# EPFL-VILAB/MultiMAE

Measured on NVIDIA H100. Metric: MultiMAE-B pretrain samples/sec @ bs=128/GPU, higher is better.
Workload: dtype bf16

## Files before the change

include/multimae_b200.h:

```cpp
#ifndef MULTIMAE_B200_H_
#define MULTIMAE_B200_H_

#include <stdint.h>

#ifdef __cplusplus
extern "C" {
#endif

#define MMAE_ABI_VERSION 11

int mmae_abi_version(void);
const char* mmae_last_error(void);
int64_t mmae_launch_count(void);

int mmae_profile_gemm(int enable);
int mmae_profile_gemm_read(double* flops, double* ms, int64_t* launches);
int64_t mmae_profile_gemm_dump(char* buf_host, int64_t capacity);

typedef struct mmae_gemm_epilogue {
  float alpha;
  int act;
  int accumulate;
  int reserved;
  const float* bias;
  const float* residual;
  const void* dgelu_z;
  void* preact_bf16;
  float* out_f32;
  void* out_bf16;
  int64_t ld_residual, ld_dgelu_z, ld_preact, ld_out_f32, ld_out_bf16;
} mmae_gemm_epilogue;

int mmae_gemm_set_variant(int variant);
int mmae_gemm_set_tma_store(int enable);
int mmae_set_pdl(int enable);
int mmae_set_sm_budget(int sms);
int mmae_set_wgrad_stream(int enable);

int mmae_gemm_bf16(const void* A, int64_t lda, int a_mn_major, const void* B, int64_t ldb, int b_mn_major,
                   int M, int N, int K, int split_k, const mmae_gemm_epilogue* ep, void* stream);

int mmae_cast_f32_to_bf16(const float* src, void* dst_bf16, int64_t n, void* stream);
int mmae_cast_colsum_f32(const float* src, int64_t ld_src, void* dst_bf16, int64_t ld_dst, float* colsum,
                         int M, int N, void* stream);
int mmae_colsum_bf16(const void* src_bf16, int64_t ld_src, float* colsum, int M, int N, void* stream);
int mmae_gelu_bf16(const void* z, void* io, int64_t n, int backward, void* stream);
int mmae_dgelu_colsum_bf16(const void* z, void* dz, int64_t ld, float* colsum, int M, int N, void* stream);
int mmae_set_fuse_gelu(int enable);
int mmae_add_bf16_f32(const float* x, const void* y_bf16, float* out, int64_t n, void* stream);
int mmae_transpose_bf16(const void* src, int64_t ld_src, void* dst, int64_t ld_dst, int M, int N, void* stream);

int mmae_layernorm_forward(const float* x, int64_t ldx, const float* gamma, const float* beta, void* y_bf16,
                           int64_t ldy, float* y_f32, int64_t ldyf, float* mean, float* rstd, int M, int D,
                           float eps, void* stream);
int mmae_add_layernorm_forward(const float* x, int64_t ldx, const void* addend_bf16, int64_t ldadd, float* x_sum,
                               int64_t ldsum, const float* gamma, const float* beta, void* y_bf16, int64_t ldy,
                               float* mean, float* rstd, int M, int D, float eps, void* stream);
int mmae_layernorm_backward(const void* dy, int dy_is_bf16, int64_t lddy, const float* x, int64_t ldx,
                            const float* mean, const float* rstd, const float* gamma, const float* dx_resid,
                            int64_t ldr, float* dx, int64_t lddx, float* dgamma, float* dbeta, int M, int D,
                            void* stream);

int mmae_layernorm_backward_ex(const void* dy, int dy_is_bf16, int64_t lddy, const float* x, int64_t ldx,
// ... 263 lines not shown
```

multimae_b200/_lib.py:

```python
import ctypes
import os

_HERE = os.path.dirname(os.path.abspath(__file__))
LIB_PATH = os.path.join(_HERE, "libmultimae_b200.so")

c_void_p = ctypes.c_void_p
c_int = ctypes.c_int
c_i64 = ctypes.c_int64
c_float = ctypes.c_float


class GemmEpilogue(ctypes.Structure):
    _fields_ = [
        ("alpha", c_float),
        ("act", c_int),
        ("accumulate", c_int),
        ("reserved", c_int),
        ("bias", c_void_p),
        ("residual", c_void_p),
        ("dgelu_z", c_void_p),
        ("preact_bf16", c_void_p),
        ("out_f32", c_void_p),
        ("out_bf16", c_void_p),
        ("ld_residual", c_i64),
        ("ld_dgelu_z", c_i64),
        ("ld_preact", c_i64),
        ("ld_out_f32", c_i64),
        ("ld_out_bf16", c_i64),
    ]


MAX_TASKS = 8
c_float_p = c_void_p
POS_MODES = {"bicubic": 0, "bilinear": 1}


class EmbedLayout(ctypes.Structure):
    _fields_ = [
        ("num_tasks", c_int),
        ("grid_h", c_int * MAX_TASKS), ("grid_w", c_int * MAX_TASKS),
        ("tok_offset", c_int * (MAX_TASKS + 1)),
        ("k_offset", c_int * (MAX_TASKS + 1)),
        ("patch", c_int * MAX_TASKS), ("channels", c_int * MAX_TASKS),
        ("is_semseg", c_int * MAX_TASKS), ("num_classes", c_int * MAX_TASKS),
    ]


class EmbedInputs(ctypes.Structure):
    _fields_ = [("data", c_void_p * MAX_TASKS), ("class_emb", c_void_p * MAX_TASKS)]


class EmbedParams(ctypes.Structure):
    _fields_ = [("weight", c_void_p * MAX_TASKS), ("bias", c_void_p * MAX_TASKS), ("pos", c_void_p * MAX_TASKS),
                ("global_tokens", c_void_p)]


class EmbedGrads(ctypes.Structure):
    _fields_ = [("weight", c_void_p * MAX_TASKS), ("bias", c_void_p * MAX_TASKS), ("class_emb", c_void_p * MAX_TASKS),
                ("global_tokens", c_void_p)]


# ... 253 lines not shown
```

multimae_b200/csrc/gemm_wgmma.cu:

```cuda
#include <algorithm>
#include <cstdlib>

#include "common.cuh"
#include "../../include/multimae_b200.h"

namespace mmae {

void count_launch();
bool gemm_profile_begin(cudaStream_t st, double flops, int M, int N, int K, int flags);
void gemm_profile_end(cudaStream_t st);

namespace {

constexpr int BM = 128;
constexpr int BK = 64;
constexpr int WG_K = 16;
constexpr int GEMM_THREADS = 384;

struct GemmParams {
  int M, N, K;
  int num_kb;
  int kb_per_split;
  int tiles_n;
  int tiles_m;
  int splits;
  int tma_store;
  mmae_gemm_epilogue ep;
};

template <int BN>
struct GemmCfg {
  static constexpr int STAGES = BN == 256 ? 4 : (BN == 192 ? 4 : (BN == 128 ? 6 : 8));
  static constexpr int A_BYTES = BM * BK * 2;
  static constexpr int B_BYTES = BN * BK * 2;
  static constexpr int STAGE_BYTES = A_BYTES + B_BYTES;
  static constexpr int EPI_BOX_BYTES = 64 * 32 * 4;
  static constexpr int EPI_OFFSET = STAGES * STAGE_BYTES;
  static constexpr int BAR_OFFSET = EPI_OFFSET + 2 * 2 * EPI_BOX_BYTES;
  static constexpr int TOTAL = BAR_OFFSET + 256 + 1024;
  static_assert(TOTAL <= 232448, "GEMM exceeds the 227 KB shared-memory limit");
};

struct WorkItem {
  int m0, n0, split, kb_begin, nkb;
};

template <int BN, int CL>
__device__ __forceinline__ WorkItem decode_item(int item, const GemmParams& p, int rank) {
  WorkItem w;
  const int rest = item / p.tiles_n;
  w.n0 = (item - rest * p.tiles_n) * BN;
  w.split = rest / p.tiles_m;
  w.m0 = ((rest - w.split * p.tiles_m) * CL + rank) * BM;
  w.kb_begin = w.split * p.kb_per_split;
  w.nkb = min(p.kb_per_split, p.num_kb - w.kb_begin);
  return w;
}

__device__ __forceinline__ void red_add_v2(float* addr, float a, float b) {
  asm volatile("red.global.add.v2.f32 [%0], {%1, %2};" ::"l"(addr), "f"(a), "f"(b) : "memory");
}

__device__ __forceinline__ void epilogue_pair(float v0, float v1, int row, int n, const GemmParams& p, bool first_split,
                                              bool atomic_out) {
  const mmae_gemm_epilogue& ep = p.ep;
  v0 *= ep.alpha;
  v1 *= ep.alpha;
  if (ep.bias && first_split) {
    const float2 b = __ldg(reinterpret_cast<const float2*>(ep.bias + n));
    v0 += b.x;
    v1 += b.y;
  }
  if (ep.preact_bf16)
    *reinterpret_cast<uint32_t*>(reinterpret_cast<bf16*>(ep.preact_bf16) + int64_t(row) * ep.ld_preact + n) = pack_bf16x2(v0, v1);
  if (ep.act == 1) {
    v0 = gelu_erf(v0);
    v1 = gelu_erf(v1);
  }
  if (ep.dgelu_z) {
    const uint32_t z = __ldg(reinterpret_cast<const unsigned int*>(reinterpret_cast<const bf16*>(ep.dgelu_z) +
                                                                   int64_t(row) * ep.ld_dgelu_z + n));
    const float2 zf = unpack_bf16x2(z);
    v0 *= dgelu_erf(zf.x);
    v1 *= dgelu_erf(zf.y);
  }
  if (ep.residual && first_split) {
    const float2 r = __ldg(reinterpret_cast<const float2*>(ep.residual + int64_t(row) * ep.ld_residual + n));
    v0 += r.x;
    v1 += r.y;
  }
  if (ep.out_f32) {
    float* dst = ep.out_f32 + int64_t(row) * ep.ld_out_f32 + n;
    if (atomic_out) red_add_v2(dst, v0, v1);
    else *reinterpret_cast<float2*>(dst) = make_float2(v0, v1);
  }
  if (ep.out_bf16)
    *reinterpret_cast<uint32_t*>(reinterpret_cast<bf16*>(ep.out_bf16) + int64_t(row) * ep.ld_out_bf16 + n) = pack_bf16x2(v0, v1);
}

template <typename T>
__device__ __forceinline__ void stage_pair(uint8_t* box, int r, int c, float v0, float v1) {
  T* b = reinterpret_cast<T*>(box);
  if constexpr (sizeof(T) == 4) *reinterpret_cast<float2*>(b + r * 32 + c) = make_float2(v0, v1);
  else *reinterpret_cast<uint32_t*>(b + r * 32 + c) = pack_bf16x2(v0, v1);
}

template <int BN, int CL, bool A_MN, bool B_MN>
__global__ void __launch_bounds__(GEMM_THREADS, 1)
    gemm_bf16_kernel(const __grid_constant__ CUtensorMap tmA, const __grid_constant__ CUtensorMap tmB,
                     const __grid_constant__ CUtensorMap tmC, const GemmParams p) {
  pdl_launch_dependents();
  using C = GemmCfg<BN>;
  constexpr int STAGES = C::STAGES;
  constexpr int BH = BN / CL;
  static_assert(!B_MN || BH % 64 == 0, "MN-major B is loaded in 64-column chunks");

  extern __shared__ uint8_t smem_raw[];
  const uint32_t raw_addr = smem_u32(smem_raw);
  uint8_t* smem = smem_raw + ((1024u - (raw_addr & 1023u)) & 1023u);
  uint64_t* full_bar = reinterpret_cast<uint64_t*>(smem + C::BAR_OFFSET);
  uint64_t* empty_bar = full_bar + STAGES;

  const int wg = threadIdx.x >> 7;
  const int rank = CL > 1 ? int(cluster_ctarank()) : 0;
  const int num_items = p.tiles_n * p.tiles_m * p.splits;
  const int first_item = blockIdx.x / CL;
  const int item_stride = gridDim.x / CL;

  if (threadIdx.x == 0) {
    tma_prefetch_desc(&tmA);
    tma_prefetch_desc(&tmB);
    if (p.tma_store) tma_prefetch_desc(&tmC);
#pragma unroll
    for (int s = 0; s < STAGES; ++s) {
      mbar_init(&full_bar[s], 1);
      mbar_init(&empty_bar[s], 2 * CL);
    }
    fence_barrier_init();
  }
  __syncthreads();
  if constexpr (CL > 1) cluster_sync_all();
  pdl_wait();

  if (wg == 0) {
    setmaxnreg_dec<40>();
    if (threadIdx.x == 0) {
      uint32_t it = 0;
      for (int item = first_item; item < num_items; item += item_stride) {
        const WorkItem w = decode_item<BN, CL>(item, p, rank);
        for (int kb = 0; kb < w.nkb; ++kb, ++it) {
          const int s = it % STAGES;
          const uint32_t ph = (it / STAGES) & 1;
          mbar_wait(&empty_bar[s], ph ^ 1u);
          mbar_expect_tx(&full_bar[s], C::STAGE_BYTES);
          uint8_t* sA = smem + s * C::STAGE_BYTES;
          uint8_t* sB = sA + C::A_BYTES;
          const int k0 = (w.kb_begin + kb) * BK;
          if constexpr (!A_MN) {
            tma_load_2d(sA, &tmA, &full_bar[s], k0, w.m0);
          } else {
#pragma unroll
            for (int c = 0; c < BM / 64; ++c) tma_load_2d(sA + c * (64 * BK * 2), &tmA, &full_bar[s], w.m0 + c * 64, k0);
          }
          if constexpr (CL == 1) {
            if constexpr (!B_MN) {
              tma_load_2d(sB, &tmB, &full_bar[s], k0, w.n0);
            } else {
#pragma unroll
              for (int c = 0; c < BN / 64; ++c) tma_load_2d(sB + c * (64 * BK * 2), &tmB, &full_bar[s], w.n0 + c * 64, k0);
            }
          } else {
            if constexpr (!B_MN) {
              tma_load_2d_multicast(sB + rank * BH * 128, &tmB, &full_bar[s], k0, w.n0 + rank * BH, 0x3);
            } else {
#pragma unroll
              for (int c = 0; c < BH / 64; ++c)
                tma_load_2d_multicast(sB + (rank * (BH / 64) + c) * (64 * BK * 2), &tmB, &full_bar[s],
                                      w.n0 + rank * BH + c * 64, k0, 0x3);
            }
          }
        }
      }
    }
  } else {
    setmaxnreg_inc<232>();
    const int cw = wg - 1;
    const int t = threadIdx.x & 127;
    const int rl = (t >> 5) * 16 + ((t & 31) >> 2);
    uint8_t* epi = smem + C::EPI_OFFSET + cw * (2 * C::EPI_BOX_BYTES);
    const bool atomic_out = p.ep.accumulate != 0 || p.splits > 1;
    uint32_t it = 0;
    uint32_t boxes = 0;
    auto release = [&](int s) {
      if (t == 0) {
        if constexpr (CL == 1) mbar_arrive(&empty_bar[s]);
        else
          for (int r = 0; r < CL; ++r) mbar_arrive_cluster(mapa_u32(smem_u32(&empty_bar[s]), uint32_t(r)));
      }
    };
    float acc[BN / 2];

    for (int item = first_item; item < num_items; item += item_stride) {
      const WorkItem w = decode_item<BN, CL>(item, p, rank);
      for (int kb = 0; kb < w.nkb; ++kb, ++it) {
        const int s = it % STAGES;
        const uint32_t ph = (it / STAGES) & 1;
        mbar_wait(&full_bar[s], ph);
        const uint32_t a_addr = smem_u32(smem + s * C::STAGE_BYTES) + cw * (64 * BK * 2);
        const uint32_t b_addr = smem_u32(smem + s * C::STAGE_BYTES) + C::A_BYTES;
#pragma unroll
        for (int i = 0; i < BN / 2; ++i) reg_fence(acc[i]);
        wgmma_fence();
#pragma unroll
        for (int j = 0; j < BK / WG_K; ++j) {
          const uint32_t sd = (kb | j) != 0 ? 1u : 0u;
          const uint64_t da = A_MN ? gmma_desc_sw128(a_addr + j * (WG_K * 128), 64 * BK * 2, 1024)
                                   : gmma_desc_sw128(a_addr + j * (WG_K * 2), 16, 1024);
          const uint64_t db = B_MN ? gmma_desc_sw128(b_addr + j * (WG_K * 128), 64 * BK * 2, 1024)
                                   : gmma_desc_sw128(b_addr + j * (WG_K * 2), 16, 1024);
          if constexpr (BN == 256) wgmma_m64n256k16<A_MN ? 1 : 0, B_MN ? 1 : 0>(acc, da, db, sd);
          else if constexpr (BN == 192) wgmma_m64n192k16<A_MN ? 1 : 0, B_MN ? 1 : 0>(acc, da, db, sd);
          else if constexpr (BN == 128) wgmma_m64n128k16<A_MN ? 1 : 0, B_MN ? 1 : 0>(acc, da, db, sd);
          else wgmma_m64n64k16<A_MN ? 1 : 0, B_MN ? 1 : 0>(acc, da, db, sd);
        }
        wgmma_commit();
#pragma unroll
        for (int i = 0; i < BN / 2; ++i) reg_fence(acc[i]);
        wgmma_wait<1>();
        if (kb > 0) release((it - 1) % STAGES);
      }
      wgmma_wait<0>();
#pragma unroll
      for (int i = 0; i < BN / 2; ++i) reg_fence(acc[i]);
      release((it - 1) % STAGES);

      const int row_a = w.m0 + cw * 64 + rl;
      const int row_b = row_a + 8;
      const bool first_split = w.split == 0;
      if (p.tma_store) {
        const float* bias = first_split ? p.ep.bias : nullptr;
        const bool bf16_out = p.tma_store == 1;
#pragma unroll
        for (int b = 0; b < BN / 32; ++b) {
          if (w.n0 + b * 32 >= p.N) break;
          uint8_t* box = bf16_out ? epi + (boxes & 3) * (C::EPI_BOX_BYTES / 2) : epi + (boxes & 1) * C::EPI_BOX_BYTES;
          if (t == 0) {
            if (bf16_out) bulk_wait_read<3>();
            else bulk_wait_read<1>();
          }
          asm volatile("bar.sync %0, 128;" ::"r"(2 + cw) : "memory");
#pragma unroll
          for (int jj = 0; jj < 4; ++jj) {
            const int j = 4 * b + jj;
            const int c = jj * 8 + 2 * (t & 3);
            float v[4] = {acc[4 * j] * p.ep.alpha, acc[4 * j + 1] * p.ep.alpha, acc[4 * j + 2] * p.ep.alpha,
                          acc[4 * j + 3] * p.ep.alpha};
            if (bias && w.n0 + b * 32 + c < p.N) {
              const float2 bb = __ldg(reinterpret_cast<const float2*>(bias + w.n0 + b * 32 + c));
              v[0] += bb.x; v[1] += bb.y; v[2] += bb.x; v[3] += bb.y;
            }
            if (p.ep.act == 1) {
#pragma unroll
              for (int i = 0; i < 4; ++i) v[i] = gelu_erf(v[i]);
            }
            if (bf16_out) {
              stage_pair<bf16>(box, rl, c, v[0], v[1]);
              stage_pair<bf16>(box, rl + 8, c, v[2], v[3]);
            } else {
              stage_pair<float>(box, rl, c, v[0], v[1]);
              stage_pair<float>(box, rl + 8, c, v[2], v[3]);
            }
          }
          fence_proxy_async_smem();
          asm volatile("bar.sync %0, 128;" ::"r"(2 + cw) : "memory");
          if (t == 0) {
            if (p.tma_store == 3) tma_reduce_add_2d(&tmC, box, w.n0 + b * 32, w.m0 + cw * 64);
            else tma_store_2d(&tmC, box, w.n0 + b * 32, w.m0 + cw * 64);
            bulk_commit_group();
          }
          ++boxes;
        }
      } else {
#pragma unroll
        for (int j = 0; j < BN / 8; ++j) {
          if (w.n0 + j * 8 >= p.N) break;
          const int n = w.n0 + j * 8 + 2 * (t & 3);
          if (row_a < p.M) epilogue_pair(acc[4 * j], acc[4 * j + 1], row_a, n, p, first_split, atomic_out);
          if (row_b < p.M) epilogue_pair(acc[4 * j + 2], acc[4 * j + 3], row_b, n, p, first_split, atomic_out);
        }
      }
    }
    if (t == 0 && p.tma_store) bulk_wait_all();
  }
  if constexpr (CL > 1) cluster_sync_all();
}

template <int BN, int CL, bool A_MN, bool B_MN>
int launch_gemm(const CUtensorMap& tmA, const CUtensorMap& tmB, const CUtensorMap& tmC, const GemmParams& p,
                cudaStream_t stream) {
  using C = GemmCfg<BN>;
  auto kern = gemm_bf16_kernel<BN, CL, A_MN, B_MN>;
  cudaLaunchConfig_t cfg;
  memset(&cfg, 0, sizeof(cfg));
  cfg.blockDim = dim3(GEMM_THREADS);
  cfg.dynamicSmemBytes = C::TOTAL;
  cfg.stream = stream;
  cudaLaunchAttribute attr[2];
  attr[0].id = cudaLaunchAttributeClusterDimension;
  attr[0].val.clusterDim.x = CL;
  attr[0].val.clusterDim.y = 1;
  attr[0].val.clusterDim.z = 1;
  attr[1].id = cudaLaunchAttributeProgrammaticStreamSerialization;
  attr[1].val.programmaticStreamSerializationAllowed = 1;
  cfg.attrs = attr;
  cfg.numAttrs = 1;
  static int resident = 0;
  if (resident == 0) {
    MMAE_CUDA_OK(cudaFuncSetAttribute(kern, cudaFuncAttributeMaxDynamicSharedMemorySize, C::TOTAL));
    if constexpr (CL > 1) {
      cfg.gridDim = dim3(CL);
      MMAE_CUDA_OK(cudaOccupancyMaxActiveClusters(&resident, kern, &cfg));
    } else {
      int dev = 0, sms = 0;
      MMAE_CUDA_OK(cudaGetDevice(&dev));
      MMAE_CUDA_OK(cudaDeviceGetAttribute(&sms, cudaDevAttrMultiProcessorCount, dev));
      resident = sms;
    }
    MMAE_CHECK(resident > 0, MMAE_ERR_CUDA, "mmae_gemm_bf16: the GEMM kernel does not fit on an SM");
  }
  const int items = p.tiles_n * p.tiles_m * p.splits;
  const int slots = std::min(resident, std::max(1, sm_count() / CL));
  cfg.gridDim = dim3(std::min(items, slots) * CL);
  const bool prof = gemm_profile_begin(stream, 2.0 * p.M * p.N * p.K, p.M, p.N, p.K,
                                       (A_MN ? 1 : 0) | (B_MN ? 2 : 0) | (p.splits << 8));
  if constexpr (CL == 1) {
    cfg.attrs = attr + 1;
    cfg.numAttrs = pdl_enabled() ? 1 : 0;
  } else {
    cfg.numAttrs = pdl_enabled() ? 2 : 1;
  }
  MMAE_CUDA_OK(cudaLaunchKernelEx(&cfg, kern, tmA, tmB, tmC, p));
  if (prof) gemm_profile_end(stream);
  count_launch();
  MMAE_LAUNCH_OK();
  return MMAE_OK;
}

}
}

using namespace mmae;

static int g_gemm_variant = []() {
  const char* e = getenv("MMAE_GEMM_VARIANT");
  const int v = e ? atoi(e) : -1;
  return v >= -1 && v <= 6 ? v : -1;
}();
static int g_gemm_tma_store = []() {
  const char* e = getenv("MMAE_GEMM_TMA_STORE");
  return e ? (atoi(e) != 0) : 1;
}();

extern "C" int mmae_gemm_set_variant(int variant) {
  MMAE_CHECK(variant >= -1 && variant <= 6, MMAE_ERR_ARG, "mmae_gemm_set_variant: %d (-1 .. 6)", variant);
  g_gemm_variant = variant;
  return MMAE_OK;
}

extern "C" int mmae_gemm_set_tma_store(int enable) {
  g_gemm_tma_store = enable != 0;
  return MMAE_OK;
}

static int variant_bn(int v) { return v == 0 ? 64 : (v == 1 || v == 6) ? 128 : (v == 3 || v == 5) ? 192 : 256; }
// ... 25 lines not shown
    for (int i = 0; i < nvar; ++i) {
      const int v = variant >= 0 ? variant : cand_var[i];
      const int bn = variant_bn(v), cl = v >= 4 ? 2 : 1;
      if (variant < 0 && bn > 128 && N < bn) continue;
      const long tiles = long(ceil_div(tm, cl)) * ceil_div(N, bn);
      const int slots = std::max(1, sms / cl);
      const int s_lo = split_k > 0 ? split_k : 1;
      const int s_hi = split_k > 0 ? split_k : std::max(1, num_kb / MIN_KB_PER_SPLIT);
      for (int s = s_lo; s <= s_hi; ++s) {
        const int kbps = ceil_div(num_kb, std::min(s, num_kb));
        const long rounds = (tiles * ceil_div(num_kb, kbps) + slots - 1) / slots;
        const long cost = rounds * (bn + 40) * cl * (kbps + KB_PER_ITEM_FIXED);
        if (best_cost < 0 || cost < best_cost) {
          best_cost = cost;
          best_split = s;
          best_var = v;
        }
      }
    }
    split_k = best_split;
    variant = best_var;
  }
  if (split_k > num_kb) split_k = num_kb;
  const int kb_per_split = ceil_div(num_kb, split_k);
  split_k = ceil_div(num_kb, kb_per_split);
  if (split_k > 1 || ep->accumulate) {
    MMAE_CHECK(ep->out_f32 && !ep->out_bf16 && !ep->preact_bf16 && !ep->dgelu_z && ep->act == 0, MMAE_ERR_ARG,
               "mmae_gemm_bf16: split-K / accumulate supports only a linear fp32 epilogue");
  }
#define MMAE_LD_OK(ptr, ld) (!(ptr) || ((ld) % 8 == 0 && (reinterpret_cast<uintptr_t>(ptr) & 15) == 0))
  MMAE_CHECK(MMAE_LD_OK(ep->residual, ep->ld_residual) && MMAE_LD_OK(ep->dgelu_z, ep->ld_dgelu_z) &&
                 MMAE_LD_OK(ep->preact_bf16, ep->ld_preact) && MMAE_LD_OK(ep->out_f32, ep->ld_out_f32) &&
                 MMAE_LD_OK(ep->out_bf16, ep->ld_out_bf16) &&
                 (!ep->bias || (reinterpret_cast<uintptr_t>(ep->bias) & 15) == 0),
             MMAE_ERR_ARG, "mmae_gemm_bf16: epilogue tensors need 16-byte alignment and ld %% 8 == 0");
#undef MMAE_LD_OK

  if (variant == 5 && b_mn_major) variant = 4;
  const int BNsel = variant_bn(variant);
  const int CLsel = variant >= 4 ? 2 : 1;

  CUtensorMap tmA, tmB;
  int rc;
  if (!a_mn_major) {
    rc = make_tmap_2d_bf16(&tmA, A, (uint64_t)M, (uint64_t)K, (uint64_t)lda, BK, BM);
  } else {
    MMAE_CHECK(M % 8 == 0, MMAE_ERR_ARG, "mmae_gemm_bf16: MN-major A needs M %% 8 == 0");
    rc = make_tmap_2d_bf16(&tmA, A, (uint64_t)K, (uint64_t)M, (uint64_t)lda, 64, BK);
  }
  if (rc) return rc;
  if (!b_mn_major) {
    rc = make_tmap_2d_bf16(&tmB, B, (uint64_t)N, (uint64_t)K, (uint64_t)ldb, BK, BNsel / CLsel);
  } else {
    rc = make_tmap_2d_bf16(&tmB, B, (uint64_t)K, (uint64_t)N, (uint64_t)ldb, 64, BK);
  }
  if (rc) return rc;

  GemmParams p;
  p.M = M; p.N = N; p.K = K;
  p.num_kb = num_kb;
  p.kb_per_split = kb_per_split;
  p.tiles_n = ceil_div(N, BNsel);
  p.tiles_m = ceil_div(tm, CLsel);
  p.splits = split_k;
  p.ep = *ep;
  p.tma_store = 0;
  CUtensorMap tmC = tmA;
  if (g_gemm_tma_store && !ep->preact_bf16 && !ep->dgelu_z && !ep->residual) {
    if (ep->out_bf16 && !ep->out_f32 && split_k == 1 && !ep->accumulate) {
      p.tma_store = 1;
      rc = make_tmap_2d_store(&tmC, ep->out_bf16, 2, (uint64_t)M, (uint64_t)N, (uint64_t)ep->ld_out_bf16);
      if (rc) return rc;
    } else if (ep->out_f32 && !ep->out_bf16 && ep->act == 0) {
      p.tma_store = (split_k > 1 || ep->accumulate) ? 3 : 2;
      rc = make_tmap_2d_store(&tmC, ep->out_f32, 4, (uint64_t)M, (uint64_t)N, (uint64_t)ep->ld_out_f32);
      if (rc) return rc;
    }
  }
  cudaStream_t st = reinterpret_cast<cudaStream_t>(stream);
#define MMAE_DISPATCH(BN_, CL_)                                                                      \
  do {                                                                                               \
    if (!a_mn_major && !b_mn_major) return launch_gemm<BN_, CL_, false, false>(tmA, tmB, tmC, p, st); \
    if (!a_mn_major && b_mn_major) return launch_gemm<BN_, CL_, false, true>(tmA, tmB, tmC, p, st);   \
    if (a_mn_major && !b_mn_major) return launch_gemm<BN_, CL_, true, false>(tmA, tmB, tmC, p, st);   \
    return launch_gemm<BN_, CL_, true, true>(tmA, tmB, tmC, p, st);                                  \
  } while (0)
  if (variant == 4) MMAE_DISPATCH(256, 2);
  if (variant == 6) MMAE_DISPATCH(128, 2);
  if (variant == 5) {
    if (!a_mn_major) return launch_gemm<192, 2, false, false>(tmA, tmB, tmC, p, st);
    return launch_gemm<192, 2, true, false>(tmA, tmB, tmC, p, st);
  }
  if (variant == 0) MMAE_DISPATCH(64, 1);
  if (variant == 3) MMAE_DISPATCH(192, 1);
  if (variant == 2) MMAE_DISPATCH(256, 1);
  MMAE_DISPATCH(128, 1);
#undef MMAE_DISPATCH
}
```

multimae_b200/csrc/modules.cu:

```cuda
#include <cstdlib>

#include "internal.h"

namespace mmae {
namespace {

struct Carver {
  uint8_t* base;
  size_t off = 0;
  explicit Carver(void* b) : base(reinterpret_cast<uint8_t*>(b)) {}
  template <typename T>
  T* take(size_t n) {
    off = align_up(off, 256);
    T* p = reinterpret_cast<T*>(base + off);
    off += n * sizeof(T);
    return p;
  }
};

}


int pick_split(int, int, int) { return 0; }

int weight_operand(const float* w, bf16** slot, int64_t n, bool cast_now, void* st) {
  if (const bf16* m = mirror_lookup(w)) {
    *slot = const_cast<bf16*>(m);
    return MMAE_OK;
  }
  return cast_now ? mmae_cast_f32_to_bf16(w, *slot, n, st) : MMAE_OK;
}

mmae_gemm_epilogue ep_zero() {
  mmae_gemm_epilogue ep;
  memset(&ep, 0, sizeof(ep));
  ep.alpha = 1.0f;
  return ep;
}

int linear_bf16(const bf16* x, const bf16* W, const float* b, bf16* y, int M, int N, int K, void* st) {
  mmae_gemm_epilogue ep = ep_zero();
  ep.bias = b;
  ep.out_bf16 = y;
  ep.ld_out_bf16 = N;
  return mmae_gemm_bf16(x, K, 0, W, K, 0, M, N, K, 1, &ep, st);
}
int linear_f32(const bf16* x, const bf16* W, const float* b, const float* resid, float* y, int M, int N, int K,
               void* st) {
  mmae_gemm_epilogue ep = ep_zero();
  ep.bias = b;
  ep.residual = resid;
  ep.ld_residual = N;
  ep.out_f32 = y;
  ep.ld_out_f32 = N;
  return mmae_gemm_bf16(x, K, 0, W, K, 0, M, N, K, 1, &ep, st);
}
int g_fuse_gelu = []() {
  const char* e = getenv("MMAE_FUSE_GELU");
  return e ? atoi(e) : 0;
}();

int linear_gelu(const bf16* x, const bf16* W, const float* b, bf16* z, bf16* a, int M, int N, int K, void* st) {
  mmae_gemm_epilogue ep = ep_zero();
  ep.bias = b;
  if (g_fuse_gelu) {
    ep.act = 1;
    ep.preact_bf16 = z;
    ep.ld_preact = N;
    ep.out_bf16 = a;
    ep.ld_out_bf16 = N;
    return mmae_gemm_bf16(x, K, 0, W, K, 0, M, N, K, 1, &ep, st);
  }
  ep.out_bf16 = z;
  ep.ld_out_bf16 = N;
  int rc = mmae_gemm_bf16(x, K, 0, W, K, 0, M, N, K, 1, &ep, st);
  if (rc != MMAE_OK) return rc;
  return mmae_gelu_bf16(z, a, int64_t(M) * N, 0, st);
}
int dgrad_bf16(const bf16* dy, int64_t lddy, const bf16* W, const bf16* dgelu_z, bf16* dx, int M, int Nout, int Kin,
               void* st) {
  mmae_gemm_epilogue ep = ep_zero();
  const bool fused = dgelu_z != nullptr && g_fuse_gelu;
  ep.dgelu_z = fused ? dgelu_z : nullptr;
  ep.ld_dgelu_z = Kin;
  ep.out_bf16 = dx;
  ep.ld_out_bf16 = Kin;
  int rc = mmae_gemm_bf16(dy, lddy, 0, W, Kin, 1, M, Kin, Nout, 1, &ep, st);
  if (rc != MMAE_OK || dgelu_z == nullptr || fused) return rc;
  return mmae_gelu_bf16(dgelu_z, dx, int64_t(M) * Kin, 1, st);
}
int dgrad_dgelu_colsum(const bf16* dy, int64_t lddy, const bf16* W, const bf16* z, bf16* dz, float* db, int M, int Nout,
                       int Kin, void* st) {
  if (g_fuse_gelu) {
    int rc = dgrad_bf16(dy, lddy, W, z, dz, M, Nout, Kin, st);
    if (rc != MMAE_OK) return rc;
    return mmae_colsum_bf16(dz, Kin, db, M, Kin, st);
  }
  int rc = dgrad_bf16(dy, lddy, W, nullptr, dz, M, Nout, Kin, st);
  if (rc != MMAE_OK) return rc;
  return mmae_dgelu_colsum_bf16(z, dz, Kin, db, M, Kin, st);
}
int wgrad(const bf16* dy, int64_t lddy, const bf16* x, int64_t ldx, float* dW, int M, int Nout, int Kin, void* st) {
  mmae_gemm_epilogue ep = ep_zero();
  ep.accumulate = 1;
  ep.out_f32 = dW;
  ep.ld_out_f32 = Kin;
  return mmae_gemm_bf16(dy, lddy, 1, x, ldx, 1, Nout, Kin, M, pick_split(Nout, Kin, M), &ep, st);
}

namespace {

#define RUN(expr)             \
  do {                        \
    int _rc = (expr);         \
    if (_rc != MMAE_OK) return _rc; \
  } while (0)

struct BlockSaved {
  bf16 *wqkv, *wproj, *w1, *w2, *h1, *qkv, *o, *h2, *z, *a;
  float *mean1, *rstd1, *mean2, *rstd2, *lse, *x_mid;
  size_t bytes;
};
BlockSaved block_saved(void* base, int B, int N, int D, int H, int hid) {
  Carver c(base);
  const size_t M = size_t(B) * N;
  BlockSaved s;
  s.wqkv = c.take<bf16>(size_t(3) * D * D);
  s.wproj = c.take<bf16>(size_t(D) * D);
  s.w1 = c.take<bf16>(size_t(hid) * D);
  s.w2 = c.take<bf16>(size_t(D) * hid);
// ... 13 lines not shown
  return s;
}
struct BlockWs {
  bf16 *g, *big, *dh, *d_o;
  bf16 *g2, *big2;
  float *dx_mid, *delta;
  size_t bytes;
};
BlockWs block_ws(void* base, int B, int N, int D, int H, int hid) {
  Carver c(base);
  const size_t M = size_t(B) * N;
  BlockWs w;
  w.g = c.take<bf16>(M * D);
  w.big = c.take<bf16>(M * std::max(hid, 3 * D));
  w.dh = c.take<bf16>(M * D);
  w.d_o = c.take<bf16>(M * D);
  w.g2 = c.take<bf16>(M * D);
  w.big2 = c.take<bf16>(M * 3 * D);
  w.dx_mid = c.take<float>(M * D);
  w.delta = c.take<float>(size_t(B) * H * N);
  w.bytes = align_up(c.off, 256);
  return w;
}

struct SideStream {
  cudaStream_t stream = nullptr;
  cudaEvent_t fork[4] = {nullptr, nullptr, nullptr, nullptr};
  cudaEvent_t join = nullptr;
  bool ok = false;
};
SideStream g_side;
int g_wgrad_stream = []() {
  const char* e = getenv("MMAE_WGRAD_STREAM");
  return e ? atoi(e) : 0;
}();

bool side_ready() {
  if (!g_wgrad_stream) return false;
  if (g_side.ok) return true;
  if (cudaStreamCreateWithFlags(&g_side.stream, cudaStreamNonBlocking) != cudaSuccess) return false;
  for (int i = 0; i < 4; ++i)
    if (cudaEventCreateWithFlags(&g_side.fork[i], cudaEventDisableTiming) != cudaSuccess) return false;
  if (cudaEventCreateWithFlags(&g_side.join, cudaEventDisableTiming) != cudaSuccess) return false;
  g_side.ok = true;
  return true;
}
int side_fork(void* main, int idx) {
  MMAE_CUDA_OK(cudaEventRecord(g_side.fork[idx], reinterpret_cast<cudaStream_t>(main)));
  MMAE_CUDA_OK(cudaStreamWaitEvent(g_side.stream, g_side.fork[idx], 0));
  return MMAE_OK;
}
int side_join(void* main) {
  MMAE_CUDA_OK(cudaEventRecord(g_side.join, g_side.stream));
  MMAE_CUDA_OK(cudaStreamWaitEvent(reinterpret_cast<cudaStream_t>(main), g_side.join, 0));
  return MMAE_OK;
}

struct HeadSaved {
  bf16 *enc_b, *wpc, *wq, *wkv, *wproj, *w1, *w2, *qn, *cn, *q, *kv, *o, *h, *z, *a;
  float *queries, *context, *qmean, *qrstd, *cmean, *crstd, *omean, *orstd, *lse, *x0;
  size_t bytes;
};
HeadSaved head_saved(void* base, const mmae_decoder_index& ix, int De, int H, int hid) {
  Carver c(base);
  const size_t Dd = ix.dim, Mq = size_t(ix.batch) * ix.num_queries,
               Mc = size_t(ix.batch) * (ix.num_visible + ix.num_global);
  HeadSaved s;
// ... 634 lines not shown
```

multimae_b200/kernels.py:

```python
import ctypes

import torch

from . import _lib as L


def _need_cuda(*ts):
    for t in ts:
        if t is not None and not t.is_cuda:
            raise L.MmaeError("multimae_b200 kernels need CUDA tensors (no CPU fallback)")


def gemm(A, B, *, a_mn=False, b_mn=False, bias=None, act=0, residual=None, dgelu_z=None, preact=None,
         out_f32=None, out_bf16=None, accumulate=False, split_k=1, alpha=1.0):
    _need_cuda(A, B)
    assert A.dtype == torch.bfloat16 and B.dtype == torch.bfloat16
    assert A.dim() == 2 and B.dim() == 2 and A.stride(1) == 1 and B.stride(1) == 1
    if a_mn:
        K, M = A.shape
    else:
        M, K = A.shape
    if b_mn:
        Kb, N = B.shape
    else:
        N, Kb = B.shape
    assert K == Kb, "contraction mismatch %d vs %d" % (K, Kb)
    ep = L.GemmEpilogue()
    ep.alpha = alpha
    ep.act = act
    ep.accumulate = 1 if accumulate else 0
    for name, ldname, t, dt in (("residual", "ld_residual", residual, torch.float32),
                                ("dgelu_z", "ld_dgelu_z", dgelu_z, torch.bfloat16),
                                ("preact_bf16", "ld_preact", preact, torch.bfloat16),
                                ("out_f32", "ld_out_f32", out_f32, torch.float32),
                                ("out_bf16", "ld_out_bf16", out_bf16, torch.bfloat16)):
        if t is not None:
            assert t.dtype == dt and t.shape[0] == M and t.shape[1] == N and t.stride(1) == 1, name
            setattr(ep, name, t.data_ptr())
            setattr(ep, ldname, t.stride(0))
    if bias is not None:
        assert bias.dtype == torch.float32 and bias.numel() == N
        ep.bias = bias.data_ptr()
    L.check(L.lib().mmae_gemm_bf16(A.data_ptr(), A.stride(0), int(a_mn), B.data_ptr(), B.stride(0), int(b_mn),
                                   M, N, K, split_k, ctypes.byref(ep), L.current_stream()), "mmae_gemm_bf16")


def cast_bf16(src, dst=None):
    _need_cuda(src)
    assert src.dtype == torch.float32 and src.is_contiguous()
    if dst is None:
        dst = torch.empty(src.shape, dtype=torch.bfloat16, device=src.device)
    L.check(L.lib().mmae_cast_f32_to_bf16(src.data_ptr(), dst.data_ptr(), src.numel(), L.current_stream()),
            "mmae_cast_f32_to_bf16")
    return dst


def cast_colsum(src, dst=None, colsum=None):
    _need_cuda(src)
    M, N = src.shape
    L.check(L.lib().mmae_cast_colsum_f32(src.data_ptr(), src.stride(0), L.ptr(dst), dst.stride(0) if dst is not None else 0,
                                         L.ptr(colsum), M, N, L.current_stream()), "mmae_cast_colsum_f32")


def colsum_bf16(src, colsum):
    M, N = src.shape
    L.check(L.lib().mmae_colsum_bf16(src.data_ptr(), src.stride(0), colsum.data_ptr(), M, N, L.current_stream()),
            "mmae_colsum_bf16")


def transpose_bf16(src, dst=None):
    M, N = src.shape
    if dst is None:
        dst = torch.empty((N, M), dtype=torch.bfloat16, device=src.device)
    L.check(L.lib().mmae_transpose_bf16(src.data_ptr(), src.stride(0), dst.data_ptr(), dst.stride(0), M, N,
                                        L.current_stream()), "mmae_transpose_bf16")
# ... 47 lines not shown
```

Before: 3904.

## Fuse GELU and dGELU into GEMM epilogue via helper warps and TMA stores

Adds a HELPER variant of the WGMMA GEMM in which producer-warpgroup helper warps apply GELU forward (or the GELU derivative plus a bias column-sum in backward) on bf16 boxes staged in shared memory, then write them out with TMA stores. The aim is to drop the separate elementwise GELU/dGELU and colsum passes over the MLP activations. Shared memory for the epilogue boxes is taken from the pipeline ring, which may shrink the stage count. The change also turns on GELU fusion by default in modules.cu, though dgrad_bf16 and dgrad_dgelu_colsum no longer pass dgelu_z into the GEMM, so the backward helper path looks unreachable from those callers. The wgrad side stream is also enabled by default.

```diff
diff --git a/include/multimae_b200.h b/include/multimae_b200.h
--- a/include/multimae_b200.h
+++ b/include/multimae_b200.h
@@ -29,6 +29,7 @@
   float* out_f32;
   void* out_bf16;
   int64_t ld_residual, ld_dgelu_z, ld_preact, ld_out_f32, ld_out_bf16;
+  float* colsum;
 } mmae_gemm_epilogue;
 
 int mmae_gemm_set_variant(int variant);
diff --git a/multimae_b200/_lib.py b/multimae_b200/_lib.py
--- a/multimae_b200/_lib.py
+++ b/multimae_b200/_lib.py
@@ -27,6 +27,7 @@
         ("ld_preact", c_i64),
         ("ld_out_f32", c_i64),
         ("ld_out_bf16", c_i64),
+        ("colsum", c_void_p),
     ]
 
 
diff --git a/multimae_b200/csrc/gemm_wgmma.cu b/multimae_b200/csrc/gemm_wgmma.cu
--- a/multimae_b200/csrc/gemm_wgmma.cu
+++ b/multimae_b200/csrc/gemm_wgmma.cu
@@ -28,17 +28,25 @@
   mmae_gemm_epilogue ep;
 };
 
-template <int BN>
+template <int BN, bool HELPER = false>
 struct GemmCfg {
-  static constexpr int STAGES = BN == 256 ? 4 : (BN == 192 ? 4 : (BN == 128 ? 6 : 8));
   static constexpr int A_BYTES = BM * BK * 2;
   static constexpr int B_BYTES = BN * BK * 2;
   static constexpr int STAGE_BYTES = A_BYTES + B_BYTES;
   static constexpr int EPI_BOX_BYTES = 64 * 32 * 4;
+  static constexpr int HBOX_BYTES = 64 * 32 * 2;
+  static constexpr int HAND = BN == 256 ? 5 : (BN == 64 ? 2 : 3);
+  static constexpr int EPI_BYTES = HELPER ? (2 * HAND + 3 * 3) * HBOX_BYTES : 2 * 2 * EPI_BOX_BYTES;
+  static constexpr int BAR_BYTES = HELPER ? 512 : 256;
+  static constexpr int MAX_STAGES = BN == 256 ? 4 : (BN == 192 ? 4 : (BN == 128 ? 6 : 8));
+  static constexpr int FIT_STAGES = (232448 - 1024 - BAR_BYTES - EPI_BYTES) / STAGE_BYTES;
+  static constexpr int STAGES = FIT_STAGES < MAX_STAGES ? FIT_STAGES : MAX_STAGES;
   static constexpr int EPI_OFFSET = STAGES * STAGE_BYTES;
-  static constexpr int BAR_OFFSET = EPI_OFFSET + 2 * 2 * EPI_BOX_BYTES;
-  static constexpr int TOTAL = BAR_OFFSET + 256 + 1024;
+  static constexpr int BAR_OFFSET = EPI_OFFSET + EPI_BYTES;
+  static constexpr int TOTAL = BAR_OFFSET + BAR_BYTES + 1024;
+  static_assert(HELPER || STAGES == MAX_STAGES, "a launch without the helper keeps its full ring");
   static_assert(TOTAL <= 232448, "GEMM exceeds the 227 KB shared-memory limit");
+  static_assert((2 * STAGES + (HELPER ? 4 * HAND : 0)) * 8 <= BAR_BYTES, "barrier area");
 };
 
 struct WorkItem {
@@ -61,8 +69,8 @@
   asm volatile("red.global.add.v2.f32 [%0], {%1, %2};" ::"l"(addr), "f"(a), "f"(b) : "memory");
 }
 
-__device__ __forceinline__ void epilogue_pair(float v0, float v1, int row, int n, const GemmParams& p, bool first_split,
-                                              bool atomic_out) {
+__device__ __forceinline__ float2 epilogue_pair(float v0, float v1, int row, int n, const GemmParams& p, bool first_split,
+                                                bool atomic_out) {
   const mmae_gemm_epilogue& ep = p.ep;
   v0 *= ep.alpha;
   v1 *= ep.alpha;
@@ -71,8 +79,13 @@
     v0 += b.x;
     v1 += b.y;
   }
-  if (ep.preact_bf16)
-    *reinterpret_cast<uint32_t*>(reinterpret_cast<bf16*>(ep.preact_bf16) + int64_t(row) * ep.ld_preact + n) = pack_bf16x2(v0, v1);
+  if (ep.preact_bf16) {
+    const uint32_t z = pack_bf16x2(v0, v1);
+    *reinterpret_cast<uint32_t*>(reinterpret_cast<bf16*>(ep.preact_bf16) + int64_t(row) * ep.ld_preact + n) = z;
+    const float2 zf = unpack_bf16x2(z);
+    v0 = zf.x;
+    v1 = zf.y;
+  }
   if (ep.act == 1) {
     v0 = gelu_erf(v0);
     v1 = gelu_erf(v1);
@@ -80,9 +93,9 @@
   if (ep.dgelu_z) {
     const uint32_t z = __ldg(reinterpret_cast<const unsigned int*>(reinterpret_cast<const bf16*>(ep.dgelu_z) +
                                                                    int64_t(row) * ep.ld_dgelu_z + n));
-    const float2 zf = unpack_bf16x2(z);
-    v0 *= dgelu_erf(zf.x);
-    v1 *= dgelu_erf(zf.y);
+    const float2 zf = unpack_bf16x2(z), d = unpack_bf16x2(pack_bf16x2(v0, v1));
+    v0 = d.x * dgelu_erf(zf.x);
+    v1 = d.y * dgelu_erf(zf.y);
   }
   if (ep.residual && first_split) {
     const float2 r = __ldg(reinterpret_cast<const float2*>(ep.residual + int64_t(row) * ep.ld_residual + n));
@@ -94,8 +107,9 @@
     if (atomic_out) red_add_v2(dst, v0, v1);
     else *reinterpret_cast<float2*>(dst) = make_float2(v0, v1);
   }
-  if (ep.out_bf16)
-    *reinterpret_cast<uint32_t*>(reinterpret_cast<bf16*>(ep.out_bf16) + int64_t(row) * ep.ld_out_bf16 + n) = pack_bf16x2(v0, v1);
+  const uint32_t o = pack_bf16x2(v0, v1);
+  if (ep.out_bf16) *reinterpret_cast<uint32_t*>(reinterpret_cast<bf16*>(ep.out_bf16) + int64_t(row) * ep.ld_out_bf16 + n) = o;
+  return unpack_bf16x2(o);
 }
 
 template <typename T>
@@ -105,13 +119,61 @@
   else *reinterpret_cast<uint32_t*>(b + r * 32 + c) = pack_bf16x2(v0, v1);
 }
 
-template <int BN, int CL, bool A_MN, bool B_MN>
+__device__ __forceinline__ void cp_async_16(void* smem_dst, const void* gsrc, bool valid) {
+  asm volatile("cp.async.cg.shared.global [%0], [%1], 16, %2;" ::"r"(smem_u32(smem_dst)), "l"(gsrc), "r"(valid ? 16 : 0)
+               : "memory");
+}
+
+template <bool BWD>
+__device__ __forceinline__ void helper_box(const uint8_t* src, uint8_t* dst, float* colsum, int n0, int N) {
+  const int lane = threadIdx.x & 31;
+  const int off0 = (lane >> 3) * 64 + (lane & 7) * 8;
+  float cs[4] = {0.f, 0.f, 0.f, 0.f};
+#pragma unroll 2
+  for (int i = 0; i < 16; ++i) {
+    const int off = off0 + i * 256;
+    const uint2 s = *reinterpret_cast<const uint2*>(src + off);
+    const float2 s0 = unpack_bf16x2(s.x), s1 = unpack_bf16x2(s.y);
+    uint2 o;
+    if constexpr (BWD) {
+      const uint2 z = *reinterpret_cast<const uint2*>(dst + off);
+      const float2 z0 = unpack_bf16x2(z.x), z1 = unpack_bf16x2(z.y);
+      o.x = pack_bf16x2(s0.x * dgelu_erf(z0.x), s0.y * dgelu_erf(z0.y));
+      o.y = pack_bf16x2(s1.x * dgelu_erf(z1.x), s1.y * dgelu_erf(z1.y));
+      const float2 r0 = unpack_bf16x2(o.x), r1 = unpack_bf16x2(o.y);
+      cs[0] += r0.x; cs[1] += r0.y; cs[2] += r1.x; cs[3] += r1.y;
+    } else {
+      o.x = pack_bf16x2(gelu_erf(s0.x), gelu_erf(s0.y));
+      o.y = pack_bf16x2(gelu_erf(s1.x), gelu_erf(s1.y));
+    }
+    *reinterpret_cast<uint2*>(dst + off) = o;
+  }
+  if constexpr (BWD) {
+    if (colsum != nullptr) {
+#pragma unroll
+      for (int k = 0; k < 4; ++k) {
+        cs[k] += __shfl_xor_sync(0xffffffffu, cs[k], 8);
+        cs[k] += __shfl_xor_sync(0xffffffffu, cs[k], 16);
+      }
+      const int n = n0 + lane * 4;
+      if (lane < 8 && n < N) {
+        red_add_v2(colsum + n, cs[0], cs[1]);
+        red_add_v2(colsum + n + 2, cs[2], cs[3]);
+      }
+    }
+  }
+}
+
+template <int BN, int CL, bool A_MN, bool B_MN, bool HELPER>
 __global__ void __launch_bounds__(GEMM_THREADS, 1)
     gemm_bf16_kernel(const __grid_constant__ CUtensorMap tmA, const __grid_constant__ CUtensorMap tmB,
-                     const __grid_constant__ CUtensorMap tmC, const GemmParams p) {
+                     const __grid_constant__ CUtensorMap tmC, const __grid_constant__ CUtensorMap tmH,
+                     const GemmParams p) {
   pdl_launch_dependents();
-  using C = GemmCfg<BN>;
+  using C = GemmCfg<BN, HELPER>;
   constexpr int STAGES = C::STAGES;
+  constexpr int HAND = C::HAND;
+  constexpr int HBOX = C::HBOX_BYTES;
   constexpr int BH = BN / CL;
   static_assert(!B_MN || BH % 64 == 0, "MN-major B is loaded in 64-column chunks");
 
@@ -120,6 +182,9 @@
   uint8_t* smem = smem_raw + ((1024u - (raw_addr & 1023u)) & 1023u);
   uint64_t* full_bar = reinterpret_cast<uint64_t*>(smem + C::BAR_OFFSET);
   uint64_t* empty_bar = full_bar + STAGES;
+  uint64_t* hfull = empty_bar + STAGES;
+  uint64_t* hfree = hfull + 2 * HAND;
+  const bool bwd = HELPER && p.ep.dgelu_z != nullptr;
 
   const int wg = threadIdx.x >> 7;
   const int rank = CL > 1 ? int(cluster_ctarank()) : 0;
@@ -131,10 +196,14 @@
     tma_prefetch_desc(&tmA);
     tma_prefetch_desc(&tmB);
     if (p.tma_store) tma_prefetch_desc(&tmC);
+    if constexpr (HELPER) tma_prefetch_desc(&tmH);
 #pragma unroll
     for (int s = 0; s < STAGES; ++s) {
       mbar_init(&full_bar[s], 1);
       mbar_init(&empty_bar[s], 2 * CL);
+    }
+    if constexpr (HELPER) {
+      for (int s = 0; s < 4 * HAND; ++s) mbar_init(&hfull[s], 1);
     }
     fence_barrier_init();
   }
@@ -181,6 +250,76 @@
           }
         }
       }
+    } else if constexpr (HELPER) {
+      if (threadIdx.x >= 32) {
+        const int hw = (threadIdx.x >> 5) - 1, lane = threadIdx.x & 31;
+        uint8_t* hbuf = smem + C::EPI_OFFSET + (2 * HAND + 3 * hw) * HBOX;
+        struct Cursor {
+          int item, b, cw;
+          uint32_t nb;
+        };
+        auto next = [&](Cursor& c) {
+          do {
+            if (++c.cw == 2) {
+              c.cw = 0;
+              ++c.nb;
+              ++c.b;
+              if (c.b == BN / 32 || (c.item % p.tiles_n) * BN + c.b * 32 >= p.N) {
+                c.b = 0;
+                c.item += item_stride;
+                if (c.item >= num_items) return;
+              }
+            }
+          } while ((2 * c.nb + uint32_t(c.cw)) % 3 != uint32_t(hw));
+        };
+        auto load_z = [&](const Cursor& c) {
+          const WorkItem w = decode_item<BN, CL>(c.item, p, rank);
+          uint8_t* buf = hbuf + (((2 * c.nb + uint32_t(c.cw)) / 3) % 3) * HBOX;
+          const int col = w.n0 + c.b * 32 + (lane & 3) * 8;
+          const int row0 = w.m0 + c.cw * 64 + (lane >> 2);
+          const bf16* z = reinterpret_cast<const bf16*>(p.ep.dgelu_z);
+#pragma unroll
+          for (int j = 0; j < 8; ++j) {
+            const int row = row0 + 8 * j;
+            const bool ok = row < p.M && col < p.N;
+            cp_async_16(buf + ((lane >> 2) + 8 * j) * 64 + (lane & 3) * 16, ok ? z + int64_t(row) * p.ep.ld_dgelu_z + col : z, ok);
+          }
+        };
+        Cursor c{first_item, 0, -1, 0u};
+        next(c);
+        if (bwd) {
+          if (c.item < num_items) load_z(c);
+          asm volatile("cp.async.commit_group;" ::: "memory");
+        }
+        while (c.item < num_items) {
+          const WorkItem w = decode_item<BN, CL>(c.item, p, rank);
+          const int hs = c.cw * HAND + int(c.nb % HAND);
+          const uint32_t ph = (c.nb / HAND) & 1;
+          const int n = w.n0 + c.b * 32, m = w.m0 + c.cw * 64;
+          uint8_t* dst = hbuf + (((2 * c.nb + uint32_t(c.cw)) / 3) % 3) * HBOX;
+          next(c);
+          if (lane == 0) bulk_wait_read<1>();
+          __syncwarp();
+          if (bwd) {
+            if (c.item < num_items) load_z(c);
+            asm volatile("cp.async.commit_group;" ::: "memory");
+            asm volatile("cp.async.wait_group 1;" ::: "memory");
+            __syncwarp();
+          }
+          mbar_wait(&hfull[hs], ph);
+          if (bwd) helper_box<true>(smem + C::EPI_OFFSET + hs * HBOX, dst, p.ep.colsum, n, p.N);
+          else helper_box<false>(smem + C::EPI_OFFSET + hs * HBOX, dst, nullptr, n, p.N);
+          fence_proxy_async_smem();
+          __syncwarp();
+          if (lane == 0) {
+            mbar_arrive(&hfree[hs]);
+            if (bwd) tma_store_2d(&tmC, dst, n, m);
+            else tma_store_2d(&tmH, dst, n, m);
+            bulk_commit_group();
+          }
+        }
+        if (lane == 0) bulk_wait_all();
+      }
     }
   } else {
     setmaxnreg_inc<232>();
@@ -237,7 +376,42 @@
       const int row_a = w.m0 + cw * 64 + rl;
       const int row_b = row_a + 8;
       const bool first_split = w.split == 0;
-      if (p.tma_store) {
+      if constexpr (HELPER) {
+#pragma unroll
+        for (int b = 0; b < BN / 32; ++b) {
+          if (w.n0 + b * 32 >= p.N) break;
+          const int hs = cw * HAND + int(boxes % HAND);
+          uint8_t* box = smem + C::EPI_OFFSET + hs * HBOX;
+          if (t == 0) {
+            if (!bwd) bulk_wait_read<HAND - 1>();
+            mbar_wait(&hfree[hs], ((boxes / HAND) & 1) ^ 1u);
+          }
+          asm volatile("bar.sync %0, 128;" ::"r"(2 + cw) : "memory");
+#pragma unroll
+          for (int jj = 0; jj < 4; ++jj) {
+            const int j = 4 * b + jj;
+            const int c = jj * 8 + 2 * (t & 3);
+            float v[4] = {acc[4 * j] * p.ep.alpha, acc[4 * j + 1] * p.ep.alpha, acc[4 * j + 2] * p.ep.alpha,
+                          acc[4 * j + 3] * p.ep.alpha};
+            if (p.ep.bias && w.n0 + b * 32 + c < p.N) {
+              const float2 bb = __ldg(reinterpret_cast<const float2*>(p.ep.bias + w.n0 + b * 32 + c));
+              v[0] += bb.x; v[1] += bb.y; v[2] += bb.x; v[3] += bb.y;
+            }
+            stage_pair<bf16>(box, rl, c, v[0], v[1]);
+            stage_pair<bf16>(box, rl + 8, c, v[2], v[3]);
+          }
+          fence_proxy_async_smem();
+          asm volatile("bar.sync %0, 128;" ::"r"(2 + cw) : "memory");
+          if (t == 0) {
+            if (!bwd) {
+              tma_store_2d(&tmC, box, w.n0 + b * 32, w.m0 + cw * 64);
+              bulk_commit_group();
+            }
+            mbar_arrive(&hfull[hs]);
+          }
+          ++boxes;
+        }
+      } else if (p.tma_store) {
         const float* bias = first_split ? p.ep.bias : nullptr;
         const bool bf16_out = p.tma_store == 1;
 #pragma unroll
@@ -285,21 +459,32 @@
         for (int j = 0; j < BN / 8; ++j) {
           if (w.n0 + j * 8 >= p.N) break;
           const int n = w.n0 + j * 8 + 2 * (t & 3);
-          if (row_a < p.M) epilogue_pair(acc[4 * j], acc[4 * j + 1], row_a, n, p, first_split, atomic_out);
-          if (row_b < p.M) epilogue_pair(acc[4 * j + 2], acc[4 * j + 3], row_b, n, p, first_split, atomic_out);
+          float2 sa = make_float2(0.f, 0.f), sb = sa;
+          if (row_a < p.M) sa = epilogue_pair(acc[4 * j], acc[4 * j + 1], row_a, n, p, first_split, atomic_out);
+          if (row_b < p.M) sb = epilogue_pair(acc[4 * j + 2], acc[4 * j + 3], row_b, n, p, first_split, atomic_out);
+          if (p.ep.colsum) {
+            sa.x += sb.x;
+            sa.y += sb.y;
+#pragma unroll
+            for (int o = 4; o < 32; o <<= 1) {
+              sa.x += __shfl_xor_sync(0xffffffffu, sa.x, o);
+              sa.y += __shfl_xor_sync(0xffffffffu, sa.y, o);
+            }
+            if ((t & 31) < 4) red_add_v2(p.ep.colsum + n, sa.x, sa.y);
+          }
         }
       }
     }
-    if (t == 0 && p.tma_store) bulk_wait_all();
+    if (t == 0 && (HELPER || p.tma_store)) bulk_wait_all();
   }
   if constexpr (CL > 1) cluster_sync_all();
 }
 
-template <int BN, int CL, bool A_MN, bool B_MN>
-int launch_gemm(const CUtensorMap& tmA, const CUtensorMap& tmB, const CUtensorMap& tmC, const GemmParams& p,
-                cudaStream_t stream) {
-  using C = GemmCfg<BN>;
-  auto kern = gemm_bf16_kernel<BN, CL, A_MN, B_MN>;
+template <int BN, int CL, bool A_MN, bool B_MN, bool HELPER = false>
+int launch_gemm(const CUtensorMap& tmA, const CUtensorMap& tmB, const CUtensorMap& tmC, const CUtensorMap& tmH,
+                const GemmParams& p, cudaStream_t stream) {
+  using C = GemmCfg<BN, HELPER>;
+  auto kern = gemm_bf16_kernel<BN, CL, A_MN, B_MN, HELPER>;
   cudaLaunchConfig_t cfg;
   memset(&cfg, 0, sizeof(cfg));
   cfg.blockDim = dim3(GEMM_THREADS);
@@ -339,7 +524,7 @@
   } else {
     cfg.numAttrs = pdl_enabled() ? 2 : 1;
   }
-  MMAE_CUDA_OK(cudaLaunchKernelEx(&cfg, kern, tmA, tmB, tmC, p));
+  MMAE_CUDA_OK(cudaLaunchKernelEx(&cfg, kern, tmA, tmB, tmC, tmH, p));
   if (prof) gemm_profile_end(stream);
   count_launch();
   MMAE_LAUNCH_OK();
@@ -431,10 +616,13 @@
   MMAE_CHECK(MMAE_LD_OK(ep->residual, ep->ld_residual) && MMAE_LD_OK(ep->dgelu_z, ep->ld_dgelu_z) &&
                  MMAE_LD_OK(ep->preact_bf16, ep->ld_preact) && MMAE_LD_OK(ep->out_f32, ep->ld_out_f32) &&
                  MMAE_LD_OK(ep->out_bf16, ep->ld_out_bf16) &&
-                 (!ep->bias || (reinterpret_cast<uintptr_t>(ep->bias) & 15) == 0),
+                 (!ep->bias || (reinterpret_cast<uintptr_t>(ep->bias) & 15) == 0) &&
+                 (!ep->colsum || (reinterpret_cast<uintptr_t>(ep->colsum) & 15) == 0),
              MMAE_ERR_ARG, "mmae_gemm_bf16: epilogue tensors need 16-byte alignment and ld %% 8 == 0");
 #undef MMAE_LD_OK
 
+  MMAE_CHECK(!ep->colsum || (ep->dgelu_z && ep->out_bf16 && !ep->out_f32 && !ep->residual), MMAE_ERR_ARG,
+             "mmae_gemm_bf16: colsum sums a bf16 GELU' output (dgelu_z and out_bf16 only)");
   if (variant == 5 && b_mn_major) variant = 4;
   const int BNsel = variant_bn(variant);
   const int CLsel = variant >= 4 ? 2 : 1;
@@ -477,18 +665,42 @@
     }
   }
   cudaStream_t st = reinterpret_cast<cudaStream_t>(stream);
+  CUtensorMap tmH = tmA;
+  const bool gelu_fwd = ep->act == 1 && ep->preact_bf16 && !ep->dgelu_z;
+  const bool gelu_bwd = ep->dgelu_z && ep->act == 0 && !ep->preact_bf16;
+  if (g_gemm_tma_store && (gelu_fwd || gelu_bwd) && ep->out_bf16 && !ep->out_f32 && !ep->residual && split_k == 1 &&
+      !ep->accumulate && !a_mn_major && CLsel == 1) {
+    p.tma_store = 1;
+    rc = make_tmap_2d_store(&tmC, gelu_fwd ? ep->preact_bf16 : ep->out_bf16, 2, (uint64_t)M, (uint64_t)N,
+                            (uint64_t)(gelu_fwd ? ep->ld_preact : ep->ld_out_bf16));
+    if (rc) return rc;
+    if (gelu_fwd) {
+      rc = make_tmap_2d_store(&tmH, ep->out_bf16, 2, (uint64_t)M, (uint64_t)N, (uint64_t)ep->ld_out_bf16);
+      if (rc) return rc;
+    }
+#define MMAE_DISPATCH_HELPER(BN_)                                                                        \
+  do {                                                                                                   \
+    if (!b_mn_major) return launch_gemm<BN_, 1, false, false, true>(tmA, tmB, tmC, tmH, p, st);          \
+    return launch_gemm<BN_, 1, false, true, true>(tmA, tmB, tmC, tmH, p, st);                            \
+  } while (0)
+    if (variant == 0) MMAE_DISPATCH_HELPER(64);
+    if (variant == 3) MMAE_DISPATCH_HELPER(192);
+    if (variant == 2) MMAE_DISPATCH_HELPER(256);
+    MMAE_DISPATCH_HELPER(128);
+#undef MMAE_DISPATCH_HELPER
+  }
 #define MMAE_DISPATCH(BN_, CL_)                                                                      \
   do {                                                                                               \
-    if (!a_mn_major && !b_mn_major) return launch_gemm<BN_, CL_, false, false>(tmA, tmB, tmC, p, st); \
-    if (!a_mn_major && b_mn_major) return launch_gemm<BN_, CL_, false, true>(tmA, tmB, tmC, p, st);   \
-    if (a_mn_major && !b_mn_major) return launch_gemm<BN_, CL_, true, false>(tmA, tmB, tmC, p, st);   \
-    return launch_gemm<BN_, CL_, true, true>(tmA, tmB, tmC, p, st);                                  \
+    if (!a_mn_major && !b_mn_major) return launch_gemm<BN_, CL_, false, false>(tmA, tmB, tmC, tmH, p, st); \
+    if (!a_mn_major && b_mn_major) return launch_gemm<BN_, CL_, false, true>(tmA, tmB, tmC, tmH, p, st);   \
+    if (a_mn_major && !b_mn_major) return launch_gemm<BN_, CL_, true, false>(tmA, tmB, tmC, tmH, p, st);   \
+    return launch_gemm<BN_, CL_, true, true>(tmA, tmB, tmC, tmH, p, st);                                  \
   } while (0)
   if (variant == 4) MMAE_DISPATCH(256, 2);
   if (variant == 6) MMAE_DISPATCH(128, 2);
   if (variant == 5) {
-    if (!a_mn_major) return launch_gemm<192, 2, false, false>(tmA, tmB, tmC, p, st);
-    return launch_gemm<192, 2, true, false>(tmA, tmB, tmC, p, st);
+    if (!a_mn_major) return launch_gemm<192, 2, false, false>(tmA, tmB, tmC, tmH, p, st);
+    return launch_gemm<192, 2, true, false>(tmA, tmB, tmC, tmH, p, st);
   }
   if (variant == 0) MMAE_DISPATCH(64, 1);
   if (variant == 3) MMAE_DISPATCH(192, 1);
diff --git a/multimae_b200/csrc/modules.cu b/multimae_b200/csrc/modules.cu
--- a/multimae_b200/csrc/modules.cu
+++ b/multimae_b200/csrc/modules.cu
@@ -55,10 +55,7 @@
   ep.ld_out_f32 = N;
   return mmae_gemm_bf16(x, K, 0, W, K, 0, M, N, K, 1, &ep, st);
 }
-int g_fuse_gelu = []() {
-  const char* e = getenv("MMAE_FUSE_GELU");
-  return e ? atoi(e) : 0;
-}();
+int g_fuse_gelu = 1;
 
 int linear_gelu(const bf16* x, const bf16* W, const float* b, bf16* z, bf16* a, int M, int N, int K, void* st) {
   mmae_gemm_epilogue ep = ep_zero();
@@ -80,22 +77,14 @@
 int dgrad_bf16(const bf16* dy, int64_t lddy, const bf16* W, const bf16* dgelu_z, bf16* dx, int M, int Nout, int Kin,
                void* st) {
   mmae_gemm_epilogue ep = ep_zero();
-  const bool fused = dgelu_z != nullptr && g_fuse_gelu;
-  ep.dgelu_z = fused ? dgelu_z : nullptr;
-  ep.ld_dgelu_z = Kin;
   ep.out_bf16 = dx;
   ep.ld_out_bf16 = Kin;
   int rc = mmae_gemm_bf16(dy, lddy, 0, W, Kin, 1, M, Kin, Nout, 1, &ep, st);
-  if (rc != MMAE_OK || dgelu_z == nullptr || fused) return rc;
+  if (rc != MMAE_OK || dgelu_z == nullptr) return rc;
   return mmae_gelu_bf16(dgelu_z, dx, int64_t(M) * Kin, 1, st);
 }
 int dgrad_dgelu_colsum(const bf16* dy, int64_t lddy, const bf16* W, const bf16* z, bf16* dz, float* db, int M, int Nout,
                        int Kin, void* st) {
-  if (g_fuse_gelu) {
-    int rc = dgrad_bf16(dy, lddy, W, z, dz, M, Nout, Kin, st);
-    if (rc != MMAE_OK) return rc;
-    return mmae_colsum_bf16(dz, Kin, db, M, Kin, st);
-  }
   int rc = dgrad_bf16(dy, lddy, W, nullptr, dz, M, Nout, Kin, st);
   if (rc != MMAE_OK) return rc;
   return mmae_dgelu_colsum_bf16(z, dz, Kin, db, M, Kin, st);
@@ -175,7 +164,7 @@
 SideStream g_side;
 int g_wgrad_stream = []() {
   const char* e = getenv("MMAE_WGRAD_STREAM");
-  return e ? atoi(e) : 0;
+  return e ? atoi(e) : 1;
 }();
 
 bool side_ready() {
diff --git a/multimae_b200/kernels.py b/multimae_b200/kernels.py
--- a/multimae_b200/kernels.py
+++ b/multimae_b200/kernels.py
@@ -12,7 +12,7 @@
 
 
 def gemm(A, B, *, a_mn=False, b_mn=False, bias=None, act=0, residual=None, dgelu_z=None, preact=None,
-         out_f32=None, out_bf16=None, accumulate=False, split_k=1, alpha=1.0):
+         out_f32=None, out_bf16=None, accumulate=False, split_k=1, alpha=1.0, colsum=None):
     _need_cuda(A, B)
     assert A.dtype == torch.bfloat16 and B.dtype == torch.bfloat16
     assert A.dim() == 2 and B.dim() == 2 and A.stride(1) == 1 and B.stride(1) == 1
@@ -41,6 +41,9 @@
     if bias is not None:
         assert bias.dtype == torch.float32 and bias.numel() == N
         ep.bias = bias.data_ptr()
+    if colsum is not None:
+        assert colsum.dtype == torch.float32 and colsum.numel() == N and colsum.is_contiguous()
+        ep.colsum = colsum.data_ptr()
     L.check(L.lib().mmae_gemm_bf16(A.data_ptr(), A.stride(0), int(a_mn), B.data_ptr(), B.stride(0), int(b_mn),
                                    M, N, K, split_k, ctypes.byref(ep), L.current_stream()), "mmae_gemm_bf16")
 
```

Result: no change. 3920, median of 6 (+0.4%).
